# swami1995/diff-qp-mpc

Hardware: AMD Instinct MI355X
Metric: QPs/sec (fwd+bwd), batch=4096 n=3 m=3 T=5 (higher is better)
Workload: dtype f64; 1 GPU; random dense QP family R (SURVEY 8d), configs[0] shape at the BASELINE metric batch: B=4096/GPU nz=30 nineq=30 neq=15; global_batch=4096, n_state=3, n_ctrl=3, T=5, parallelism=batch-shard x1, termination=batch (the reference's batch-coupled rule, parity-safe)

## Files before the change

diff-qp-mpc_amd/_lib.py:

```python
import ctypes
import os
import re

import torch

from . import _build


class dqp_dims(ctypes.Structure):
    _fields_ = [("nbatch", ctypes.c_int32), ("nz", ctypes.c_int32), ("nineq", ctypes.c_int32),
                ("neq", ctypes.c_int32),
                ("stride_Q", ctypes.c_int64), ("stride_p", ctypes.c_int64),
                ("stride_G", ctypes.c_int64), ("stride_h", ctypes.c_int64),
                ("stride_A", ctypes.c_int64), ("stride_b", ctypes.c_int64)]


class dqp_opts(ctypes.Structure):
    _fields_ = [("eps", ctypes.c_double), ("stall_tol", ctypes.c_double),
                ("max_iter", ctypes.c_int32),
                ("not_improved_lim", ctypes.c_int32), ("flags", ctypes.c_uint32),
                ("reserved", ctypes.c_int32),
                ("dyn_id", ctypes.c_int32), ("dyn_T", ctypes.c_int32), ("dyn_dt", ctypes.c_double),
                ("dyn_x0", ctypes.c_void_p)]


DQP_OK = 0
DQP_FLAG_DENSE_BACKWARD = 1
DQP_FLAG_GENERIC_ONLY = 2
DQP_FLAG_NO_NULLSPACE = 4
DQP_FLAG_RIC_GLOBAL_WS = 64
DQP_FLAG_BACKWARD_CTX = 8
DQP_FLAG_BATCH_TERMINATION = 16
DQP_FLAG_HISTORY_ONLY = 32
DQP_FLAG_STRICT_GET_STEP = 128
DQP_FLAG_STAGEWISE = 256
DQP_STATUS_Q_NOT_PD = 1
DQP_STATUS_A_RANK_DEF = 2
DQP_MAX_DIM = 64
DQP_MAX_DIM_LARGE = 512
SHARED_GRAD_KC = 64


class dqp_al_mpc_dims(ctypes.Structure):
    _fields_ = [("nbatch", ctypes.c_int32), ("n_state", ctypes.c_int32), ("n_ctrl", ctypes.c_int32),
                ("T", ctypes.c_int32)]


class dqp_al_bounds(ctypes.Structure):
    _fields_ = [("lower", ctypes.c_void_p), ("upper", ctypes.c_void_p), ("stride_b", ctypes.c_int64),
                ("stride_t", ctypes.c_int64)]


class dqp_al_dims(ctypes.Structure):
    _fields_ = [("nbatch", ctypes.c_int32), ("nz", ctypes.c_int32), ("ncon", ctypes.c_int32),
                ("reserved", ctypes.c_int32)]


class dqp_mpc_dims(ctypes.Structure):
    _fields_ = [("nbatch", ctypes.c_int32), ("n_state", ctypes.c_int32), ("n_ctrl", ctypes.c_int32),
                ("T", ctypes.c_int32), ("has_bounds", ctypes.c_int32), ("dyn_id", ctypes.c_int32),
                ("n_state_host", ctypes.c_int32)]


class dqp_deq_dims(ctypes.Structure):
    _fields_ = [("nrows", ctypes.c_int32), ("hdim", ctypes.c_int32)]


class dqp_trace_record(ctypes.Structure):
# ... 139 lines not shown
```

diff-qp-mpc_amd/csrc/dqp_common.h:

```cpp
#ifndef DQP_COMMON_H_
#define DQP_COMMON_H_
#include <hip/hip_runtime.h>
#include <stdint.h>

#include "../../include/dqp.h"
#include "dqp_trace.h"

namespace dqp {

constexpr int WAVE = 64;

struct KParams {
    const double *Q, *p, *G, *h, *A, *b;
    long long sQ, sp, sG, sh, sA, sb;
    double *zhat, *lam, *nu, *slack, *best_resid;
    const double *zin, *lamin, *nuin, *slackin, *gin;
    double *dQ, *dp, *dG, *dh, *dA, *db;
    int32_t *info;
    double *workspace;
    unsigned long long *stamps;
    int B, N, M, E;
    int ldz, ldm, lde, ldt;
    double eps, stallTol;
    int maxIter, notImprovedLim;
    unsigned flags;
    double *hist;
    const int32_t *cap;
    int histIters;
    int dynId, dynT, dynN, dynM;
    double dynDt;
    const double *dynX0;
    const double *mC, *mc, *mF, *mf, *mx0, *mul, *muu;
    double *mdC, *mdc, *mdF, *mdf, *mdx0;
    int mn, mm, mT;
    double *snap;
    const double *histIn;
    const double *extRy;
    int itBegin, itEnd;
};

__host__ __device__ inline long long mpc_bound_stride_b(const KParams &P) { return P.sG; }
__host__ __device__ inline long long mpc_bound_stride_t(const KParams &P) { return P.sh; }
inline bool mpc_bounds_strided(const KParams &P) { return P.sG != 0 || P.sh != 0; }
inline void mpc_set_bounds(KParams &P, const dqp_al_bounds *b)
{
    P.mul = b->lower; P.muu = b->upper; P.sG = b->stride_b; P.sh = b->stride_t;
}

constexpr int TERM_HDR = 8;

constexpr int TERM_MAXIT = 64;
constexpr int TERM_ACC_BYTES = 3 * 8 + TERM_HDR * 4;

__device__ __forceinline__ void hist_put(const KParams &P, long long qp, int it, double resid, double mu)
{
    double2 *h = reinterpret_cast<double2 *>(P.hist) + (long long)it * P.B + qp;
    *h = make_double2(resid, mu);
}
__device__ __forceinline__ void hist_fill(const KParams &P, long long qp, int iters)
{
    const double nan = __builtin_nan("");
    for (int it = iters; it < P.histIters; ++it)
        reinterpret_cast<double2 *>(P.hist)[(long long)it * P.B + qp] = make_double2(nan, nan);
}
__device__ __forceinline__ void term_zero_acc(const KParams &P)
{
    if (P.hist && blockIdx.x == 0) {
        unsigned *a = reinterpret_cast<unsigned *>(P.hist + (long long)P.B * P.histIters * 2);
        for (int i = threadIdx.x; i < TERM_ACC_BYTES / 4; i += blockDim.x) a[i] = 0u;
    }
}

__device__ __forceinline__ int rule_stop(unsigned long long ai, unsigned long long anb, unsigned long long ana, int maxIter,
                                         int notImprovedLim)
{
    int nNot = 0;
    for (int it = 0; it < maxIter; ++it) {
        if (it == 0 || ((ai >> it) & 1ull)) nNot = 0;
        else nNot += 1;
        if (nNot == notImprovedLim || !((anb >> it) & 1ull) || !((ana >> it) & 1ull)) return it + 1;
    }
    return maxIter;
}

__device__ __forceinline__ unsigned long long term_uniform(unsigned long long v)
{
    const unsigned lo = __builtin_amdgcn_readfirstlane((unsigned)v), hi = __builtin_amdgcn_readfirstlane((unsigned)(v >> 32));
    return ((unsigned long long)hi << 32) | lo;
}

template <bool SCALAR = false> __device__ __forceinline__ int term_cap(const KParams &P)
{
    const unsigned long long *m =
        reinterpret_cast<const unsigned long long *>(reinterpret_cast<const char *>(P.cap) - (TERM_ACC_BYTES - TERM_HDR * 4));
    const int c = P.cap[0];
    unsigned long long ai = m[0], anb = m[1], ana = m[2];
    if (SCALAR) {
        ai = term_uniform(ai); anb = term_uniform(anb); ana = term_uniform(ana);
        asm volatile("" : "+s"(ai), "+s"(anb), "+s"(ana));
    } else {
        asm volatile("" : "+v"(ai), "+v"(anb), "+v"(ana));
    }
    if (c > 0) return c;
    const int istar = rule_stop(ai, anb, ana, P.maxIter, P.notImprovedLim);
    if (blockIdx.x == 0 && threadIdx.x == 0) const_cast<int32_t *>(P.cap)[0] = istar;
    return istar;
}

__device__ __forceinline__ int term_best(const KParams &P, long long qp) { return P.cap[TERM_HDR + qp]; }
__device__ __forceinline__ bool term_flagged(const KParams &P, long long qp, int cap) { return term_best(P, qp) >= cap; }

size_t term_bytes(int B, int maxIter, int snapDim);
int term_decide(const KParams &P, void *term, void *stream);
int term_local_masks(const KParams &P, void *term, unsigned long long *masks, void *stream);
int term_decide_global(const KParams &P, void *term, const unsigned long long *masks, void *stream);
void term_bind_pass1(KParams &P, void *term, int snapDim);
void term_bind_pass2(KParams &P, void *term);


#ifdef DQP_STAMPS
extern unsigned long long *g_debug_stamps;
#endif
int r16_forward(const KParams &P, void *stream);
int r16_backward(const KParams &P, void *stream);
int r16n_forward(const KParams &P, void *stream);
long long r16n_workspace_doubles(int N, int M, int E);
int r16n_snapshot_doubles(int N, int M, int E);
bool stage_supported(int n_state, int n_ctrl);
bool stage_native(int n_state, int n_ctrl);
int stage_q(int n_state, int n_ctrl);
long long stage_layout_doubles(int n_state, int n_ctrl, int T);
int stage_snapshot_doubles(int n_state, int n_ctrl, int T);
long long stage_workspace_doubles(int n_state, int n_ctrl, int T, int B, bool stepped);
int stage_forward(const KParams &P, void *stream);
int stage_forward_stepped(const KParams &P, void *stream);
int stage_backward(const KParams &P, void *stream);
int stage_finish(const KParams &P, void *stream);
enum { STAGE_FORWARD = 0, STAGE_STEPPED = 1, STAGE_BACKWARD = 2 };
struct PadRegion {
    double *C, *F, *c, *tau, *g, *dc, *f, *df, *nu, *ry, *x0, *dx0, *dC, *dF;
};
long long pad_region_doubles(int n_host, int n_ctrl, int T, int B);
PadRegion pad_region(double *base, int n_host, int n_ctrl, int T, int B);
int pad_pack(int n, int n_host, int m, int T, int B, const PadRegion &R, const double *C, const double *c, const double *F,
             const double *f, const double *x0, const double *tau, const double *nu, const double *g, const double *ry,
             void *stream);
int pad_unpack(int n, int n_host, int m, int T, int B, const PadRegion &R, double *tau, double *nu, double *dC, double *dc,
               double *dF, double *df, double *dx0, void *stream);
long long big_workspace_doubles(int N, int M, int E);
bool big_fits(int N, int M, int E);
// ... 11 lines not shown
```

diff-qp-mpc_amd/csrc/dqp_mpc_qp.hip:

```cpp
#include "dqp_common.h"
#include "dqp_al_bounds.h"
#include "dqp_dyn_models.h"

using namespace dqp;

namespace {

struct Route {
    bool stage;
    bool padded;
};

struct Io {
    const double *C, *c, *F, *f, *x0;
    const dqp_mpc_bounds *bounds;
    double *tau, *lam, *nu, *slack;
    int32_t *info;
    double *best_resid;
    void *workspace, *termination;
    bool complete() const
    {
        return C && c && F && f && x0 && bounds->lower && bounds->upper && tau && lam && nu && slack && workspace;
    }
};
// ... 68 lines not shown
int forward(const dqp_mpc_dims *md, const dqp_opts *opts, KParams &P, Route rt, bool stepped, const Io &io, void *stream)
{
    int rc;
    P.mC = io.C; P.mc = io.c; P.mF = io.F; P.mf = io.f; P.mx0 = io.x0;
    mpc_set_bounds(P, io.bounds);
    P.zhat = io.tau; P.lam = io.lam; P.nu = io.nu; P.slack = io.slack; P.info = io.info; P.best_resid = io.best_resid;
    P.workspace = (double *)io.workspace;
    const bool batch = (P.flags & DQP_FLAG_BATCH_TERMINATION) != 0;
    if (batch && (!io.termination || P.maxIter > 64)) return DQP_ERR_BAD_ARG;
    const bool first = !stepped || P.itBegin == 0, last = !stepped || P.itEnd == P.maxIter;
    PadRegion R = {};
    if (rt.padded) {
        R = pad_region(P.workspace + stage_workspace_doubles(P.mn, P.mm, P.mT, P.B, stepped), P.mn, P.mm, P.mT, P.B);
        const double *ry = P.itEnd > P.itBegin ? P.extRy : nullptr;
        rc = pad_pack(md->n_state, P.mn, P.mm, P.mT, P.B, R, first ? io.C : nullptr, first ? io.c : nullptr,
                      first ? io.F : nullptr, first ? io.f : nullptr, first ? io.x0 : nullptr, nullptr, nullptr, nullptr, ry,
                      stream);
        if (rc != DQP_OK) return rc;
        P.mC = R.C; P.mc = R.c; P.mF = R.F; P.mf = R.f; P.mx0 = R.x0; P.zhat = R.tau; P.nu = R.nu;
        P.extRy = ry ? R.ry : nullptr;
    }
    auto done = [&](int r) {
        if (r != DQP_OK || !rt.padded) return r;
        return pad_unpack(md->n_state, P.mn, P.mm, P.mT, P.B, R, io.tau, last ? io.nu : nullptr, nullptr, nullptr, nullptr,
                          nullptr, nullptr, stream);
    };
    if (batch) {
        P.eps = opts ? opts->eps : 1e-12;
        term_bind_pass1(P, io.termination, snapshot_doubles(P, rt));
    }
    rc = !rt.stage ? r16n_forward(P, stream) : stepped ? stage_forward_stepped(P, stream) : stage_forward(P, stream);
    if (rc != DQP_OK) return stepped && rc == 1 ? DQP_ERR_TOO_LARGE : rc;
    if (!batch || !last || (P.flags & DQP_FLAG_HISTORY_ONLY)) return done(DQP_OK);
    if ((rc = term_decide(P, io.termination, stream)) != DQP_OK) return rc;
    term_bind_pass2(P, io.termination);
    return done(rt.stage ? stage_finish(P, stream) : r16n_forward(P, stream));
}

}

extern "C" {

__attribute__((visibility("default"))) size_t dqp_mpc_qp_termination_bytes(const dqp_mpc_dims *md, const dqp_opts *o)
{
    KParams P = {};
    size_t lds = 0;
    Route rt;
    if (!o || !(o->flags & DQP_FLAG_BATCH_TERMINATION) || mpc_params(md, o, P, lds, rt) != DQP_OK || md->nbatch <= 0) return 0;
    return term_bytes(P.B, P.maxIter, snapshot_doubles(P, rt));
}

__attribute__((visibility("default"))) int dqp_mpc_qp_supported(const dqp_mpc_dims *md)
{
    KParams P = {};
    size_t lds = 0;
    Route rt;
    return mpc_params(md, nullptr, P, lds, rt) == DQP_OK ? 1 : 0;
}

__attribute__((visibility("default"))) size_t dqp_mpc_qp_workspace_bytes(const dqp_mpc_dims *md)
{
    KParams P = {};
    size_t lds = 0;
    Route rt;
    if (mpc_params(md, nullptr, P, lds, rt) != DQP_OK || md->nbatch <= 0) return 0;
    return workspace_doubles(P, rt, false) * sizeof(double);
}

// ... 123 lines not shown
```

diff-qp-mpc_amd/csrc/dqp_pdipm.hip:

```cpp

#include <hip/hip_runtime.h>
#include <math.h>
#include <stdint.h>

#include "dqp_common.h"
#include "dqp_al_bounds.h"
#include "dqp_dyn_models.h"

using namespace dqp;

namespace {

#define WSYNC() __syncthreads()

__device__ __forceinline__ double bcast(double v, int src)
{
    int lo = __double2loint(v), hi = __double2hiint(v);
    lo = __builtin_amdgcn_readlane(lo, src);
    hi = __builtin_amdgcn_readlane(hi, src);
    return __hiloint2double(hi, lo);
}

template <int CTRL> __device__ __forceinline__ double dppd(double v)
{
// ... 575 lines not shown
            const double dni = bcast(dnu, i), ni = bcast(nu, i);
            if (inN) o[i * N + lane] = dni * zh + ni * dx;
        }
    }
    if (lane == 0 && P.info) { P.info[2 * qp] = status; P.info[2 * qp + 1] = 0; }
}

template <typename K>
int launch(K kernel, const KParams &P, size_t lds_bytes, void *stream)
{
    if (P.B == 0) return DQP_OK;
    if (lds_bytes > 64 * 1024) {
        if (hipFuncSetAttribute(reinterpret_cast<const void *>(kernel),
                                hipFuncAttributeMaxDynamicSharedMemorySize,
                                (int)lds_bytes) != hipSuccess)
            return DQP_ERR_LAUNCH;
    }
    DQP_LAUNCH(kernel, dim3(P.B), dim3(WAVE), lds_bytes, (hipStream_t)stream, P);
    return hipGetLastError() == hipSuccess ? DQP_OK : DQP_ERR_LAUNCH;
}

}

static inline bool is_big(const KParams &P) { return P.N > DQP_MAX_DIM || P.M > DQP_MAX_DIM || P.E > DQP_MAX_DIM; }

namespace dqp {

void fill_opts(const dqp_opts *o, KParams &P)
{
    P.eps = (o ? o->eps : 1e-12) * 0.1;
    P.stallTol = o ? o->stall_tol : 1e-10;
    P.maxIter = o ? o->max_iter : 20;
    P.notImprovedLim = o ? o->not_improved_lim : 3;
    P.flags = o ? o->flags : 0u;
    P.hist = nullptr; P.cap = nullptr; P.histIters = P.maxIter;
}

int fill_params(const dqp_dims *d, const dqp_opts *o, KParams &P, size_t &lds_bytes)
{
#ifdef DQP_STAMPS
    P.stamps = dqp::g_debug_stamps;
#else
    P.stamps = nullptr;
#endif
    if (!d) return DQP_ERR_BAD_ARG;
    if (d->nbatch < 0 || d->nz <= 0 || d->nineq <= 0 || d->neq < 0) return DQP_ERR_BAD_ARG;
    if (d->nz > DQP_MAX_DIM_LARGE || d->nineq > DQP_MAX_DIM_LARGE || d->neq > DQP_MAX_DIM_LARGE) return DQP_ERR_TOO_LARGE;
    P.B = d->nbatch; P.N = d->nz; P.M = d->nineq; P.E = d->neq;
    if (is_big(P)) {
        if (!big_fits(P.N, P.M, P.E)) return DQP_ERR_TOO_LARGE;
        if (o && o->dyn_id) return DQP_ERR_BAD_ARG;
        P.sQ = d->stride_Q; P.sp = d->stride_p; P.sG = d->stride_G;
        P.sh = d->stride_h; P.sA = d->stride_A; P.sb = d->stride_b;
        fill_opts(o, P);
        lds_bytes = 0;
        return DQP_OK;
    }
    P.ldz = d->nz | 1; P.ldm = d->nineq | 1; P.lde = d->neq | 1;
    P.ldt = P.ldz > P.ldm ? P.ldz : P.ldm;
    P.sQ = d->stride_Q; P.sp = d->stride_p; P.sG = d->stride_G;
    P.sh = d->stride_h; P.sA = d->stride_A; P.sb = d->stride_b;
    fill_opts(o, P);
    P.dynId = o ? o->dyn_id : 0;
    P.dynT = 0; P.dynN = 0; P.dynM = 0; P.dynDt = 0.0; P.dynX0 = nullptr;
    if (P.dynId) {
        int32_t n = 0, m = 0;
        if (dqp_dyn_sizes(P.dynId, &n, &m) != DQP_OK) return DQP_ERR_BAD_ARG;
// ... 62 lines not shown

static int bind_forward(KParams &P, const double *Q, const double *p, const double *G, const double *h, const double *A,
                        const double *b, double *zhat, double *lam, double *nu, double *slack, int32_t *info,
                        double *best_resid, void *workspace)
{
    if (!Q || !p || !G || !h || !zhat || !lam || !slack) return DQP_ERR_BAD_ARG;
    if (P.E > 0 && (!A || !b || !nu)) return DQP_ERR_BAD_ARG;
    P.Q = Q; P.p = p; P.G = G; P.h = h; P.A = A; P.b = b;
    P.zhat = zhat; P.lam = lam; P.nu = nu; P.slack = slack;
    P.info = info; P.best_resid = best_resid;
    P.workspace = (double *)workspace;
    return DQP_OK;
}

__attribute__((visibility("default"))) int
dqp_qp_forward(const dqp_dims *dims, const dqp_opts *opts, const double *Q, const double *p,
               const double *G, const double *h, const double *A, const double *b, double *zhat,
               double *lam, double *nu, double *slack, int32_t *info, double *best_resid,
               void *workspace, void *termination, void *stream)
{
    KParams P = {};
    size_t lds = 0;
    int rc = fill_params(dims, opts, P, lds);
    if (rc != DQP_OK) return rc;
    if (P.B == 0) return DQP_OK;
    if ((rc = bind_forward(P, Q, p, G, h, A, b, zhat, lam, nu, slack, info, best_resid, workspace)) != DQP_OK) return rc;
    if (!(P.flags & DQP_FLAG_BATCH_TERMINATION)) return forward_once(P, lds, workspace, stream);
    if (!termination || P.maxIter < 1 || P.maxIter > 64) return DQP_ERR_BAD_ARG;
    P.eps = opts ? opts->eps : 1e-12;
    const bool nullspace = workspace && !(P.flags & (DQP_FLAG_GENERIC_ONLY | DQP_FLAG_NO_NULLSPACE)) && !P.dynId && !is_big(P);
    term_bind_pass1(P, termination, nullspace ? r16n_snapshot_doubles(P.N, P.M, P.E) : 0);
    if ((rc = forward_once(P, lds, workspace, stream)) != DQP_OK) return rc;
    if (P.flags & DQP_FLAG_HISTORY_ONLY) return DQP_OK;
    if ((rc = term_decide(P, termination, stream)) != DQP_OK) return rc;
    term_bind_pass2(P, termination);
    return forward_once(P, lds, workspace, stream);
}

__attribute__((visibility("default"))) int
dqp_term_local_masks(const dqp_dims *dims, const dqp_opts *opts, void *termination, uint64_t *masks, void *stream)
{
    KParams P = {};
    size_t lds = 0;
    int rc = fill_params(dims, opts, P, lds);
    if (rc != DQP_OK) return rc;
    if (!(P.flags & DQP_FLAG_BATCH_TERMINATION) || !termination || !masks || P.maxIter < 1 || P.maxIter > 64)
        return DQP_ERR_BAD_ARG;
    if (P.B == 0) return hipMemsetAsync(masks, 0, 24, (hipStream_t)stream) == hipSuccess ? DQP_OK : DQP_ERR_LAUNCH;
    P.eps = opts ? opts->eps : 1e-12;
    return term_local_masks(P, termination, (unsigned long long *)masks, stream);
}

__attribute__((visibility("default"))) int
dqp_qp_forward_finish(const dqp_dims *dims, const dqp_opts *opts, const double *Q, const double *p,
                      const double *G, const double *h, const double *A, const double *b, double *zhat,
                      double *lam, double *nu, double *slack, int32_t *info, double *best_resid,
                      void *workspace, void *termination, const uint64_t *masks, void *stream)
{
    KParams P = {};
    size_t lds = 0;
    int rc = fill_params(dims, opts, P, lds);
    if (rc != DQP_OK) return rc;
    if (P.B == 0) return DQP_OK;
    if (!(P.flags & DQP_FLAG_BATCH_TERMINATION) || !termination || !masks || P.maxIter < 1 || P.maxIter > 64)
        return DQP_ERR_BAD_ARG;
    if ((rc = bind_forward(P, Q, p, G, h, A, b, zhat, lam, nu, slack, info, best_resid, workspace)) != DQP_OK) return rc;
    P.eps = opts ? opts->eps : 1e-12;
    const bool nullspace = workspace && !(P.flags & (DQP_FLAG_GENERIC_ONLY | DQP_FLAG_NO_NULLSPACE)) && !P.dynId && !is_big(P);
// ... 55 lines not shown
```

diff-qp-mpc_amd/csrc/dqp_r16n.hip:

```cpp

#include "dqp_r16_prims.h"

namespace dqp {
namespace r16n {

using namespace dqp::r16;

#ifndef DQP_PF_REFLECT
#define DQP_PF_REFLECT DQP_LDS_PREFETCH
#endif
#ifndef DQP_PF_ROWS
#define DQP_PF_ROWS DQP_LDS_PREFETCH
#endif
#ifndef DQP_PF_HEADS
#define DQP_PF_HEADS DQP_LDS_PREFETCH
#endif

template <int N_, int M_, int E_> struct Cfg {
    static constexpr int N = N_, M = M_, E = E_, R = N_ - E_;
    static constexpr int SN = slots(N_), SM = slots(M_), SR = slots(N_ - E_);
    static constexpr int SE = E_ > 0 ? slots(E_) : 1, EC = E_ > 0 ? E_ : 1;
    static constexpr bool PARK = slots(N_) >= 3;
    static constexpr bool PF = !PARK;
    static constexpr int RING = (PF && DQP_PF_TRI) ? DQP_TRI_RING : 0;
// ... 7 lines not shown
#endif
    static constexpr bool PIN = PARK || DQP_R16N_PIN_ALL;
#ifndef DQP_R16N_SPLIT_ALL
#define DQP_R16N_SPLIT_ALL 0
#endif
    static constexpr bool SPLIT = PARK || DQP_R16N_SPLIT_ALL;
#ifndef DQP_R16N_EARLY_CTX
#define DQP_R16N_EARLY_CTX 1
#endif
    static constexpr bool EARLY = DQP_R16N_EARLY_CTX;
    static constexpr int tailsz = E_ * (N_ - E_) + E_ * (E_ - 1) / 2;
    static constexpr int oLq = 0;
    static constexpr int oTl = tri(N_);
    static constexpr int oR = oTl;
    static constexpr int shared = tailsz > tri(M_) ? tailsz : tri(M_);
    static constexpr int oCp = oTl + shared;
    static constexpr int oHp = oCp + (N_ - E_);
    static constexpr int oQv = oHp + M_;
    static constexpr int oBw = oQv + N_;
    static constexpr int oBs = oBw + (N_ - E_), oBz = oBs + M_, oBc = oBz + M_;
    static constexpr int oDummy = oBc + 2;
    static constexpr int ldsQP = oDummy + 16;
    static constexpr int ldsQPpad = (ldsQP + 1) & ~1;
#ifndef DQP_R16N_STAGED
#define DQP_R16N_STAGED 0
#endif
    static constexpr bool STAGED = DQP_R16N_STAGED && 16 * N_ <= ldsQP - oTl;
    __host__ __device__ static constexpr int toff(int k) { return k * (N_ - E_) + k * (k - 1) / 2; }
    static constexpr int wTl = 0, wLq = tailsz, wG = wLq + tri(N_), wU = wG + M_ * N_;
    static constexpr int wTau = wU + E_ * E_, wRdu = wTau + E_, wRdq = wRdu + E_;
    static constexpr int wXy = wRdq + N_, wPy = wXy + E_, wW1 = wPy + E_, wDl = wW1 + E_;
    static constexpr int wsQP = wDl + 1;
    static constexpr int snapDim = (N_ - E_) + 2 * M_ + 2;
};

#define DQP_PHASE_FENCE() asm volatile("" ::: "memory")
__device__ __forceinline__ void pin(double &x) { asm volatile("" : "+v"(x) : : "memory"); }
__device__ __forceinline__ const double *relabel(const double *p)
{
    asm volatile("" : "+v"(p));
    return p;
}

template <class C> struct State {
    double Gh[C::SM][C::N];
    double LqZ[C::SN][C::R];
    double Ah[C::SE][C::N];
    double tau[C::SE];
    double rdu1[C::SE];
    double xy[C::SE];
    double py[C::SE];
    double w1[C::SE];
    double rdq[C::SN];
    double rdiag[C::SM];
    int status;
};

template <class C>
__device__ __forceinline__ void shift_down(const double (&vn)[C::SN], double (&ve)[C::SE], int r)
{
#pragma unroll
    for (int s = 0; s < C::SE; ++s) ve[s] = 0.0;
#pragma unroll
    for (int e = 0; e < C::E; ++e) {
        const double t = BC(vn, C::R + e);
        if (r == (e & 15)) ve[e >> 4] = t;
// ... 886 lines not shown
            if (inM[s]) { P.lam[qp * M + r + 16 * s] = bz[s]; P.slack[qp * M + r + 16 * s] = bs[s]; }
        if (E > 0) {
#pragma unroll
            for (int s = 0; s < SE; ++s)
                if (r + 16 * s < E) P.nu[qp * E + r + 16 * s] = yv[s];
        }
        if (r == 0) {
            if (P.info) { P.info[2 * qp] = st.status; P.info[2 * qp + 1] = iters; }
            if (P.best_resid) P.best_resid[qp] = best;
        }
    }
}

template <class C>
__global__ __launch_bounds__(64) void forward_kernel(KParams P)
{
    constexpr int N = C::N, M = C::M, E = C::E, R = C::R;
    constexpr int SN = C::SN, SM = C::SM, SE = C::SE, SR = C::SR;
    extern __shared__ __attribute__((aligned(16))) double sm[];
    const int lane = threadIdx.x, r = lane & 15, qrow = lane >> 4;
    long long qp = (long long)blockIdx.x * 4 + qrow;
    bool live = qp < P.B;
    if (!live) qp = P.B - 1;
    int maxIter = P.maxIter;
    const bool batch = (P.flags & DQP_FLAG_BATCH_TERMINATION) != 0;
    const bool strict = (P.flags & DQP_FLAG_STRICT_GET_STEP) != 0;
    if (P.cap) {
        const int cap = term_cap<true>(P);
        maxIter = min(maxIter, cap);
        live = live && term_flagged(P, qp, cap);
        if (__builtin_amdgcn_ballot_w64(live) == 0) return;
    }
    double *lds = sm + qrow * C::ldsQPpad;
    double *dummy = lds + C::oDummy + r;

    term_zero_acc(P);
    State<C> st;
    STAMP(P, 0);
    setup<C>(P, qp, r, lds, st);
    STAMP(P, 15);

    bool inM[SM], inR[SR];
#pragma unroll
    for (int s = 0; s < SM; ++s) inM[s] = r + 16 * s < M;
#pragma unroll
    for (int s = 0; s < SR; ++s) inR[s] = r + 16 * s < R;

    double T[SM][M], rdu[SM];
    double w[SR], s_[SM], z[SM];
    double cc = 1.0, delta = 0.0;
    {
        double one[SM], hp[SM], cp[SR], g[SM], gtz[SR];
#pragma unroll
        for (int s = 0; s < SM; ++s) one[s] = inM[s] ? 1.0 : 0.0;
        vec_get<SM>(lds + C::oHp, hp, M, r);
        vec_get<SR>(lds + C::oCp, cp, R, r);
        mul_Gz<C>(st, cp, g);
#pragma unroll
        for (int s = 0; s < SM; ++s) g[s] = inM[s] ? -hp[s] - g[s] : 0.0;
        __builtin_amdgcn_sched_barrier(0);
        factor_T_rhs<C>(lds, T, st.rdiag, one, rdu, g, r);
        __builtin_amdgcn_sched_barrier(0);
        mul_GzT<C>(st, g, gtz, r);
#pragma unroll
        for (int s = 0; s < SR; ++s) w[s] = inR[s] ? -cp[s] - gtz[s] : 0.0;
        double ms = INFINITY, mz = INFINITY;
// ... 31 lines not shown
#pragma unroll
            for (int s = 0; s < SR; ++s) rw[s] = inR[s] ? w[s] + cp[s] + gz[s] : 0.0;
#pragma unroll
            for (int s = 0; s < SM; ++s) rz[s] = inM[s] ? gw[s] + s_[s] - hp[s] : 0.0;
        }
        double sz = 0.0, nz2 = 0.0;
#pragma unroll
        for (int s = 0; s < SM; ++s) { sz = fma(s_[s], z[s], sz); nz2 = fma(rz[s], rz[s], nz2); }
        double nx2 = rx_norm2_partial<C>(st, lds, rw, cc * delta, r);
        sz = row_sum(sz); nz2 = row_sum(nz2); nx2 = row_sum(nx2);
        const double mu = fabs(sz * (1.0 / M));
        const double resid = sqrt(nz2) + sqrt(nx2) + M * mu;
        if (!done) {
            iters = it + 1;
            if (!have_best || resid < best) {
                nNot = 0; have_best = true; best = resid; bestc = cc;
                vec_put<SR>(lds + C::oBw, w, R, r, dummy);
                vec_put<SM>(lds + C::oBs, s_, M, r, dummy);
                vec_put<SM>(lds + C::oBz, z, M, r, dummy);
                if (P.snap && live) {
                    double *sp = P.snap + ((long long)it * P.B + qp) * C::snapDim;
#pragma unroll
                    for (int s = 0; s < SR; ++s)
                        if (inR[s]) sp[r + 16 * s] = w[s];
#pragma unroll
                    for (int s = 0; s < SM; ++s)
                        if (inM[s]) { sp[R + r + 16 * s] = s_[s]; sp[R + M + r + 16 * s] = z[s]; }
                    if (r == 0) sp[R + 2 * M] = cc;
                }
            } else {
                nNot += 1;
            }
            if (batch) {
                if (P.hist && r == 0 && live) hist_put(P, qp, it, resid, mu);
                done = !(fabs(resid) < INFINITY);
            } else if ((nNot >= P.notImprovedLim && best < P.stallTol) || best < P.eps || mu > 1e32 ||
                       !(fabs(resid) < INFINITY))
                done = true;
        }
        if (__builtin_amdgcn_ballot_w64(!done) == 0 || it + 1 >= maxIter) break;
        if (it == 1) STAMP(P, 9);

        double dza[SM], dsa[SM];
        {
            double gu[SM];
            mul_Gz<C>(st, rw, gu);
#pragma unroll
            for (int s = 0; s < SM; ++s) dza[s] = rz[s] - s_[s] - gu[s];
        }
        __builtin_amdgcn_sched_barrier(0);
        double dinv[SM];
#pragma unroll
        for (int s = 0; s < SM; ++s) dinv[s] = inM[s] ? s_[s] * frcp(z[s]) : 0.0;
        factor_T_rhs<C>(lds, T, st.rdiag, dinv, rdu, dza, r);
        if (it == 1) STAMP(P, 10);
        if (it == 1) STAMP(P, 11);
        double rzv[SM], rsv[SM];
#pragma unroll
        for (int s = 0; s < SM; ++s) {
            rzv[s] = inM[s] ? frcp(z[s]) : 0.0;
            rsv[s] = inM[s] ? frcp(s_[s]) : 0.0;
        }
        double tm = 0.0;
#pragma unroll
        for (int s = 0; s < SM; ++s) {
            dsa[s] = (-z[s] - dza[s]) * dinv[s];
            tm = fmax(tm, fmax(-dza[s] * rzv[s], -dsa[s] * rsv[s]));
// ... 21 lines not shown
        if (it == 1) STAMP(P, 12);
        tm = 0.0;
#pragma unroll
        for (int s = 0; s < SM; ++s) {
            dz[s] = dza[s] + dzc[s];
            ds[s] = fma(-rsc[s] - dzc[s], dinv[s], dsa[s]);
            tm = fmax(tm, fmax(-dz[s] * rzv[s], -ds[s] * rsv[s]));
        }
        if (strict) {
#pragma unroll
            for (int s = 0; s < SM; ++s) zero_step |= inM[s] && (dz[s] == 0.0 || ds[s] == 0.0);
            if ((__builtin_amdgcn_ballot_w64(zero_step) >> (lane & 48)) & 0xffffull) done = true;
        }
        __builtin_amdgcn_sched_barrier(0);
        double gtd[SR];
        mul_GzT<C>(st, dz, gtd, r);
        alpha = frcp(fmax(row_max(tm) * (1.0 / 0.999), 1.0));
        if (!done) {
#pragma unroll
            for (int s = 0; s < SR; ++s) {
                w[s] = fma(alpha, -rw[s] - gtd[s], w[s]);
                gz[s] = fma(alpha, gtd[s], gz[s]);
            }
#pragma unroll
            for (int s = 0; s < SM; ++s) { s_[s] = fma(alpha, ds[s], s_[s]); z[s] = fma(alpha, dz[s], z[s]); }
            cc *= (1.0 - alpha);
        }
        if (it == 1) STAMP(P, 13);
        if (it == 0) STAMP(P, 8);
    }
    STAMP(P, 7);

    if (P.hist && r == 0 && live) hist_fill(P, qp, iters);
    epilogue<C>(P, qp, r, lds, st, bestc, delta, iters, best, live, true);
    STAMP(P, 14);
}

template <class C>
__device__ __forceinline__ void load_ctx(const KParams &P, long long qp, int r, double *lds, State<C> &st)
{
    constexpr int N = C::N, M = C::M, E = C::E, R = C::R;
    constexpr int SN = C::SN, SM = C::SM, SE = C::SE;
    st.status = DQP_STATUS_OK;
    {
        const double *ws = P.workspace + qp * (long long)C::wsQP;
        CtxRegs<C::tailsz> tl;
        CtxRegs<tri(N)> lq;
        ctx_fetch<C::tailsz>(ws + C::wTl, tl, r);
        ctx_fetch<tri(N)>(ws + C::wLq, lq, r);
        ctx_stash<C::tailsz>(lds + C::oTl, tl, r);
        ctx_stash<tri(N)>(lds + C::oLq, lq, r);
#pragma unroll
        for (int s = 0; s < SM; ++s) {
            const int i = r + 16 * s, ic = i < M ? i : M - 1;
#pragma unroll
            for (int c = 0; c < N; ++c) {
                const double v = ws[C::wG + c * M + ic];
                st.Gh[s][c] = (16 * s + 15 >= M) ? mask_hi(v, i < M) : v;
            }
        }
#pragma unroll
        for (int s = 0; s < SE; ++s) {
            const int k = r + 16 * s, kc = k < E ? k : E - 1;
#pragma unroll
            for (int c = 0; c < N; ++c) st.Ah[s][c] = 0.0;
#pragma unroll
            for (int e = 0; e < E; ++e) {
                const double v = ws[C::wU + e * E + kc];
                st.Ah[s][R + e] = k < E ? v : 0.0;
            }
            const double t = ws[C::wTau + kc], u = ws[C::wRdu + kc];
            st.tau[s] = k < E ? t : 0.0;
            st.rdu1[s] = k < E ? u : 0.0;
        }
#pragma unroll
        for (int s = 0; s < SN; ++s) {
            const int i = r + 16 * s;
            const double v = ws[C::wRdq + (i < N ? i : N - 1)];
            st.rdq[s] = i < N ? v : 0.0;
        }
    }
}

template <class C>
__global__ __launch_bounds__(64) void finish_kernel(KParams P)
{
    constexpr int M = C::M, E = C::E, R = C::R;
    constexpr int SM = C::SM, SE = C::SE, SR = C::SR;
    extern __shared__ __attribute__((aligned(16))) double sm[];
    const int lane = threadIdx.x, r = lane & 15, qrow = lane >> 4;
    long long qp = (long long)blockIdx.x * 4 + qrow;
    bool live = qp < P.B;
    if (!live) qp = P.B - 1;
    const int mine = term_best(P, qp);
    const int istar = term_cap<true>(P);
    live = live && mine >= istar;
    if (__builtin_amdgcn_ballot_w64(live) == 0) return;
    const int cap = min(P.maxIter, istar);
    double *lds = sm + qrow * C::ldsQPpad;
    double *dummy = lds + C::oDummy + r;
    State<C> st;
    load_ctx<C>(P, qp, r, lds, st);
    const double *ws = P.workspace + qp * (long long)C::wsQP;
#pragma unroll
    for (int s = 0; s < SE; ++s) {
        const int k = r + 16 * s, kc = k < E ? k : (E > 0 ? E - 1 : 0);
        const double a = ws[C::wXy + kc], b = ws[C::wPy + kc], c = ws[C::wW1 + kc];
        st.xy[s] = (E > 0 && k < E) ? a : 0.0;
        st.py[s] = (E > 0 && k < E) ? b : 0.0;
        st.w1[s] = (E > 0 && k < E) ? c : 0.0;
    }
    const double delta = ws[C::wDl];
    const double2 *h = reinterpret_cast<const double2 *>(P.histIn) + qp;
    double hv[64];
#pragma unroll
    for (int it = 0; it < 64; ++it) hv[it] = h[(long long)(it < cap ? it : 0) * P.B].x;
    double best = hv[0];
    int arg = 0;
#pragma unroll
    for (int it = 1; it < 64; ++it)
        if (it < cap && hv[it] < best) { best = hv[it]; arg = it; }
    const double *sp = P.snap + ((long long)arg * P.B + qp) * C::snapDim;
    double bw[SR], bs[SM], bz[SM];
#pragma unroll
    for (int s = 0; s < SR; ++s) { const int i = r + 16 * s; const double v = sp[i < R ? i : 0]; bw[s] = i < R ? v : 0.0; }
#pragma unroll
    for (int s = 0; s < SM; ++s) {
        const int i = r + 16 * s, ic = i < M ? i : 0;
// ... 167 lines not shown
        double *o = P.dQ + qp * N * N;
#pragma unroll
        for (int i = 0; i < N; ++i) {
            const double dxi = BC(dxh, i), zi = BC(zh, i);
#pragma unroll
            for (int s = 0; s < SN; ++s)
                if (inN[s]) o[i * N + r + 16 * s] = 0.5 * (dxi * zh[s] + zi * dxh[s]);
        }
    }
    if (P.dG) {
        double *o = P.dG + qp * M * N;
#pragma unroll
        for (int i = 0; i < M; ++i) {
            const double dli = BC(dlam, i), li = BC(lam, i);
#pragma unroll
            for (int s = 0; s < SN; ++s)
                if (inN[s]) o[i * N + r + 16 * s] = dli * zh[s] + li * dxh[s];
        }
    }
    if (P.dA && E > 0) {
        double *o = P.dA + qp * E * N;
#pragma unroll
        for (int i = 0; i < E; ++i) {
            const double dni = BC(dnu, i), ni = BC(nu, i);
#pragma unroll
            for (int s = 0; s < SN; ++s)
                if (inN[s]) o[i * N + r + 16 * s] = dni * zh[s] + ni * dxh[s];
        }
    }
    if (r == 0 && P.info) { P.info[2 * qp] = st.status; P.info[2 * qp + 1] = 0; }
}

template <class C, class K>
int launch(K kernel, const KParams &P, void *stream)
{
    const size_t lds = (size_t)4 * C::ldsQPpad * sizeof(double);
    if (lds > 64 * 1024 &&
        hipFuncSetAttribute(reinterpret_cast<const void *>(kernel),
                            hipFuncAttributeMaxDynamicSharedMemorySize, (int)lds) != hipSuccess)
        return DQP_ERR_LAUNCH;
    const int blocks = (P.B + 3) / 4;
    DQP_LAUNCH(kernel, dim3(blocks), dim3(64), lds, (hipStream_t)stream, P);
    return hipGetLastError() == hipSuccess ? DQP_OK : DQP_ERR_LAUNCH;
}

}

#if !defined(DQP_R16_N) || !defined(DQP_R16_M) || !defined(DQP_R16_E)
#error "compile with -DDQP_R16_N=.. -DDQP_R16_M=.. -DDQP_R16_E=.."
#endif
#define DQP_CAT2(a, n, m, e) a##n##_##m##_##e
#define DQP_CAT(a, n, m, e) DQP_CAT2(a, n, m, e)

#ifndef DQP_R16_BWD
int DQP_CAT(r16n_forward_, DQP_R16_N, DQP_R16_M, DQP_R16_E)(const KParams &P, void *stream)
{
    using C = r16n::Cfg<DQP_R16_N, DQP_R16_M, DQP_R16_E>;
    if (P.cap && P.snap && P.histIn) return r16n::launch<C>(r16n::finish_kernel<C>, P, stream);
    return r16n::launch<C>(r16n::forward_kernel<C>, P, stream);
}
#else
int DQP_CAT(r16n_backward_, DQP_R16_N, DQP_R16_M, DQP_R16_E)(const KParams &P, void *stream)
{
    using C = r16n::Cfg<DQP_R16_N, DQP_R16_M, DQP_R16_E>;
    return r16n::launch<C>(r16n::backward_kernel<C>, P, stream);
}
#endif

}
```

diff-qp-mpc_amd/csrc/dqp_term.hip:

```cpp
#include "dqp_common.h"

namespace dqp {

namespace {

constexpr int MAXIT = TERM_MAXIT;
struct Acc {
    unsigned long long improved;
    unsigned long long notbelow;
    unsigned long long notabove;
};
static_assert(sizeof(Acc) + TERM_HDR * sizeof(int32_t) == TERM_ACC_BYTES, "layout shared with dqp_common.h");

inline size_t hist_bytes(int B, int maxIter) { return (size_t)B * maxIter * 2 * sizeof(double); }

__device__ __forceinline__ unsigned long long wave_or_u64(unsigned long long v)
{
#pragma unroll
    for (int off = 32; off > 0; off >>= 1) v |= __shfl_xor(v, off, 64);
    return v;
}

constexpr int SCAN_CHUNK = 32;
__global__ __launch_bounds__(64) void term_scan_kernel(const double2 *hist, Acc *acc, int32_t *hdr,
                                                       int B, int maxIter, double eps)
{
    const int lane = threadIdx.x;
    const long long qp = (long long)blockIdx.x * blockDim.x + lane;
    const bool live = qp < B;
    unsigned long long imp = 0ull, nb = 0ull, na = 0ull;
    if (live) {
        const double2 *h = hist + qp;
        double best = 0.0;
        int arg = 0;
        for (int it0 = 0; it0 < maxIter; it0 += SCAN_CHUNK) {
            double2 v[SCAN_CHUNK];
#pragma unroll
            for (int k = 0; k < SCAN_CHUNK; ++k) v[k] = h[(long long)min(it0 + k, maxIter - 1) * B];
#pragma unroll
            for (int k = 0; k < SCAN_CHUNK; ++k) {
                const int it = it0 + k;
                if (it < maxIter) {
                    if (it == 0) best = v[k].x;
                    else if (v[k].x < best) { best = v[k].x; arg = it; imp |= 1ull << it; }
                    if (!(best < eps)) nb |= 1ull << it;
                    if (!(v[k].y > 1e32)) na |= 1ull << it;
                }
            }
        }
        hdr[TERM_HDR + qp] = arg;
    }
    imp = wave_or_u64(imp); nb = wave_or_u64(nb); na = wave_or_u64(na);
    if (lane < 3) {
        const unsigned long long m = lane == 0 ? imp : (lane == 1 ? nb : na);
        unsigned long long *dst = lane == 0 ? &acc->improved : (lane == 1 ? &acc->notbelow : &acc->notabove);
        if (m) atomicOr(dst, m);
    }
}

__global__ __launch_bounds__(64) void term_decide_kernel(const unsigned long long *masks, int32_t *hdr, int maxIter,
                                                         int notImprovedLim)
{
    if (threadIdx.x == 0) hdr[0] = rule_stop(masks[0], masks[1], masks[2], maxIter, notImprovedLim);
}

inline Acc *acc_of(void *term, int B, int maxIter) { return (Acc *)((char *)term + hist_bytes(B, maxIter)); }
inline int32_t *hdr_of(void *term, int B, int maxIter) { return (int32_t *)((char *)acc_of(term, B, maxIter) + sizeof(Acc)); }

inline size_t snap_offset(int B, int maxIter)
{
    const size_t o = hist_bytes(B, maxIter) + sizeof(Acc) + (size_t)(TERM_HDR + B) * sizeof(int32_t);
    return (o + 15) & ~(size_t)15;
}

}

size_t term_bytes(int B, int maxIter, int snapDim)
{
    if (B <= 0 || maxIter <= 0) return 0;
    return snap_offset(B, maxIter) + (size_t)B * maxIter * (snapDim > 0 ? snapDim : 0) * sizeof(double);
}

void term_bind_pass1(KParams &P, void *term, int snapDim)
{
    P.hist = (double *)term;
    P.histIters = P.maxIter;
    P.cap = nullptr;
    P.histIn = nullptr;
    P.snap = snapDim > 0 ? (double *)((char *)term + snap_offset(P.B, P.maxIter)) : nullptr;
}

void term_bind_pass2(KParams &P, void *term)
{
    P.hist = nullptr;
    P.histIn = (const double *)term;
    P.cap = hdr_of(term, P.B, P.maxIter);
}

int term_decide(const KParams &P, void *term, void *stream)
{
    const int blocks = (P.B + 63) / 64;
    DQP_LAUNCH(term_scan_kernel, dim3(blocks), dim3(64), 0, (hipStream_t)stream,
                       (const double2 *)term, acc_of(term, P.B, P.maxIter), hdr_of(term, P.B, P.maxIter),
                       P.B, P.maxIter, P.eps);
    return hipGetLastError() == hipSuccess ? DQP_OK : DQP_ERR_LAUNCH;
}

int term_local_masks(const KParams &P, void *term, unsigned long long *masks, void *stream)
{
    const int blocks = (P.B + 63) / 64;
    DQP_LAUNCH(term_scan_kernel, dim3(blocks), dim3(64), 0, (hipStream_t)stream,
                       (const double2 *)term, acc_of(term, P.B, P.maxIter), hdr_of(term, P.B, P.maxIter),
                       P.B, P.maxIter, P.eps);
    if (hipMemcpyAsync(masks, acc_of(term, P.B, P.maxIter), 3 * sizeof(unsigned long long), hipMemcpyDeviceToDevice,
                       (hipStream_t)stream) != hipSuccess)
        return DQP_ERR_LAUNCH;
    return hipGetLastError() == hipSuccess ? DQP_OK : DQP_ERR_LAUNCH;
}

int term_decide_global(const KParams &P, void *term, const unsigned long long *masks, void *stream)
{
    DQP_LAUNCH(term_decide_kernel, dim3(1), dim3(64), 0, (hipStream_t)stream, masks,
                       hdr_of(term, P.B, P.maxIter), P.maxIter, P.notImprovedLim);
    return hipGetLastError() == hipSuccess ? DQP_OK : DQP_ERR_LAUNCH;
}

// ... 2 lines not shown
```

include/dqp.h:

```cpp
#ifndef DQP_H_
#define DQP_H_

#include <stddef.h>
#include <stdint.h>

#ifdef __cplusplus
extern "C" {
#endif

#define DQP_VERSION 303
#define DQP_MAX_DIM 64
#define DQP_MAX_DIM_LARGE 512

enum {
    DQP_OK = 0,
    DQP_ERR_BAD_ARG = -1,
    DQP_ERR_TOO_LARGE = -2,
    DQP_ERR_LAUNCH = -3,
    DQP_ERR_NO_DEVICE = -4
};

enum {
    DQP_STATUS_OK = 0,
    DQP_STATUS_Q_NOT_PD = 1,
    DQP_STATUS_A_RANK_DEF = 2
};

#define DQP_FLAG_DENSE_BACKWARD 1u

#define DQP_FLAG_GENERIC_ONLY 2u
#define DQP_FLAG_BACKWARD_CTX 8u
#define DQP_FLAG_BATCH_TERMINATION 16u
#define DQP_FLAG_HISTORY_ONLY 32u
#define DQP_FLAG_NO_NULLSPACE 4u
#define DQP_FLAG_RIC_GLOBAL_WS 64u

#define DQP_FLAG_STRICT_GET_STEP 128u

#define DQP_FLAG_STAGEWISE 256u

typedef struct dqp_dims {
    int32_t nbatch;
    int32_t nz;
    int32_t nineq;
    int32_t neq;
    int64_t stride_Q, stride_p, stride_G, stride_h, stride_A, stride_b;
} dqp_dims;

typedef struct dqp_opts {
    double eps;
    double stall_tol;
    int32_t max_iter;
    int32_t not_improved_lim;
    uint32_t flags;
    int32_t reserved;
    int32_t dyn_id;
    int32_t dyn_T;
    double dyn_dt;
    const double *dyn_x0;
} dqp_opts;

int dqp_version(void);
const char *dqp_error_string(int code);


size_t dqp_workspace_bytes(const dqp_dims *dims);

size_t dqp_termination_bytes(const dqp_dims *dims, const dqp_opts *opts);

int dqp_term_local_masks(const dqp_dims *dims, const dqp_opts *opts, void *termination, uint64_t *masks,
                         void *stream);
int dqp_qp_forward_finish(const dqp_dims *dims, const dqp_opts *opts, const double *Q, const double *p,
// ... 312 lines not shown
```

Measured before the change: 18.15 million QPs/sec.

## Fuse batch-termination scan into forward kernel tail via LDS history and per-wave slots

The forward kernel now records each problem's residual and mu history in LDS instead of global memory. At the end of the kernel it computes the per-problem termination masks and argmin, then writes wave-ORed mask slots to global memory. The finish kernel ORs those slots to decide the stopping iteration, so the separate term_scan kernel launch is skipped for small-N nullspace configs. This saves a launch and a strided history re-read, at the cost of extra LDS per block, which could reduce occupancy, and more complex sync between waves.

```diff
diff --git a/diff-qp-mpc_amd/_lib.py b/diff-qp-mpc_amd/_lib.py
--- a/diff-qp-mpc_amd/_lib.py
+++ b/diff-qp-mpc_amd/_lib.py
@@ -34,6 +34,7 @@
 DQP_FLAG_HISTORY_ONLY = 32
 DQP_FLAG_STRICT_GET_STEP = 128
 DQP_FLAG_STAGEWISE = 256
+DQP_FLAG_TERM_SCAN = 512
 DQP_STATUS_Q_NOT_PD = 1
 DQP_STATUS_A_RANK_DEF = 2
 DQP_MAX_DIM = 64
diff --git a/diff-qp-mpc_amd/csrc/dqp_common.h b/diff-qp-mpc_amd/csrc/dqp_common.h
--- a/diff-qp-mpc_amd/csrc/dqp_common.h
+++ b/diff-qp-mpc_amd/csrc/dqp_common.h
@@ -52,6 +52,67 @@
 constexpr int TERM_MAXIT = 64;
 constexpr int TERM_ACC_BYTES = 3 * 8 + TERM_HDR * 4;
 
+#ifndef DQP_TERM_SLOT_WAVES
+#define DQP_TERM_SLOT_WAVES 1024
+#endif
+constexpr unsigned TERM_FLAG_SLOTS = 1u << 31;
+constexpr bool r16n_term_lds(int N) { return (N + 15) / 16 < 3; }
+
+struct TermMasks {
+    unsigned long long improved;
+    unsigned long long notbelow;
+    unsigned long long notabove;
+    int arg;
+};
+template <int CHUNK>
+__host__ __device__ inline TermMasks term_problem_masks(const double2 *h, long long stride, int maxIter, double eps)
+{
+    TermMasks m = {0ull, 0ull, 0ull, 0};
+    double best = 0.0;
+    for (int it0 = 0; it0 < maxIter; it0 += CHUNK) {
+        double2 v[CHUNK];
+#pragma unroll
+        for (int k = 0; k < CHUNK; ++k) {
+            const int itc = it0 + k < maxIter ? it0 + k : maxIter - 1;
+            v[k] = h[(long long)itc * stride];
+        }
+#pragma unroll
+        for (int k = 0; k < CHUNK; ++k) {
+            const int it = it0 + k;
+            if (it < maxIter) {
+                if (it == 0) best = v[k].x;
+                else if (v[k].x < best) { best = v[k].x; m.arg = it; m.improved |= 1ull << it; }
+                if (!(best < eps)) m.notbelow |= 1ull << it;
+                if (!(v[k].y > 1e32)) m.notabove |= 1ull << it;
+            }
+        }
+    }
+    return m;
+}
+
+__host__ __device__ inline int term_slot_pairs(int W) { return (W + 1) >> 1; }
+__host__ __device__ inline size_t term_slot_bytes(int W) { return (size_t)3 * term_slot_pairs(W) * 16; }
+template <int ROUNDS>
+__host__ __device__ inline unsigned long long term_slot_or(const unsigned long long *slots, int W, int run, int first,
+                                                           int lane, int nlanes)
+{
+    const int np = term_slot_pairs(W);
+    const ulonglong2 *s = reinterpret_cast<const ulonglong2 *>(slots) + (long long)run * np;
+    ulonglong2 v[ROUNDS];
+    bool odd[ROUNDS];
+#pragma unroll
+    for (int k = 0; k < ROUNDS; ++k) {
+        const int j = first + lane + k * nlanes, jc = j < np ? j : np - 1;
+        v[k] = s[jc];
+        odd[k] = 2 * jc + 1 >= W;
+    }
+    unsigned long long o = 0ull;
+#pragma unroll
+    for (int k = 0; k < ROUNDS; ++k) o |= v[k].x | (odd[k] ? 0ull : v[k].y);
+    return o;
+}
+constexpr int TERM_SLOT_ROUNDS = 8;
+
 __device__ __forceinline__ void hist_put(const KParams &P, long long qp, int it, double resid, double mu)
 {
     double2 *h = reinterpret_cast<double2 *>(P.hist) + (long long)it * P.B + qp;
@@ -107,6 +168,90 @@
     return istar;
 }
 
+__device__ __forceinline__ unsigned long long term_lane(unsigned long long v, int l)
+{
+    const unsigned lo = __builtin_amdgcn_readlane((unsigned)v, l), hi = __builtin_amdgcn_readlane((unsigned)(v >> 32), l);
+    return ((unsigned long long)hi << 32) | lo;
+}
+__device__ __forceinline__ unsigned term_row_or(unsigned v)
+{
+    v |= (unsigned)__builtin_amdgcn_update_dpp((int)v, (int)v, 0x128, 0xf, 0xf, true);
+    v |= (unsigned)__builtin_amdgcn_update_dpp((int)v, (int)v, 0x124, 0xf, 0xf, true);
+    v |= (unsigned)__builtin_amdgcn_update_dpp((int)v, (int)v, 0x122, 0xf, 0xf, true);
+    v |= (unsigned)__builtin_amdgcn_update_dpp((int)v, (int)v, 0x121, 0xf, 0xf, true);
+    return v;
+}
+__device__ __forceinline__ unsigned long long term_wave_or(unsigned long long v)
+{
+    const unsigned long long w = ((unsigned long long)term_row_or((unsigned)(v >> 32)) << 32) | term_row_or((unsigned)v);
+    return term_lane(w, 0) | term_lane(w, 16) | term_lane(w, 32) | term_lane(w, 48);
+}
+
+__host__ __device__ inline size_t term_slot_offset(int B, int maxIter, int snapDim)
+{
+    return (((size_t)B * maxIter * snapDim * sizeof(double)) + 15) & ~(size_t)15;
+}
+__device__ __forceinline__ unsigned long long *term_slots(const KParams &P, int snapDim)
+{
+    return reinterpret_cast<unsigned long long *>(reinterpret_cast<char *>(P.snap) + term_slot_offset(P.B, P.maxIter, snapDim));
+}
+
+__device__ __forceinline__ void term_pass1_tail(const KParams &P, double2 *hl, int qstride, long long qp, bool live, int iters,
+                                                int snapDim)
+{
+    int lane = __builtin_amdgcn_mbcnt_hi(~0u, __builtin_amdgcn_mbcnt_lo(~0u, 0u)), maxIter = P.maxIter;
+    asm volatile("" : "+v"(lane), "+s"(maxIter));
+    const int r = lane & 15, qrow = lane >> 4;
+    double2 *mine = hl + qrow * qstride;
+    if (r == 0) {
+        const double nan = __builtin_nan("");
+        for (int it = iters; it < maxIter; ++it) mine[it] = make_double2(nan, nan);
+    }
+    {
+        const long long qp0 = (long long)blockIdx.x * 4;
+        const int q = lane & 3;
+        double2 *g = reinterpret_cast<double2 *>(P.hist) + qp0 + q;
+#pragma unroll
+        for (int k = 0; k < TERM_MAXIT / 16; ++k) {
+            const int it = (lane >> 2) + 16 * k;
+            if (it < maxIter && qp0 + q < P.B) g[(long long)it * P.B] = hl[q * qstride + it];
+        }
+    }
+    TermMasks m = {0ull, 0ull, 0ull, 0};
+    if (r == 0 && live) {
+        m = term_problem_masks<8>(mine, 1, maxIter, P.eps);
+        reinterpret_cast<int32_t *>(P.hist + (long long)P.B * P.histIters * 2)[TERM_ACC_BYTES / 4 + qp] = m.arg;
+    }
+    if (P.snap) {
+        const int W = (P.B + 3) >> 2, np = term_slot_pairs(W);
+        const unsigned long long a = term_lane(m.improved, 0) | term_lane(m.improved, 16) | term_lane(m.improved, 32) |
+                                     term_lane(m.improved, 48);
+        const unsigned long long b = term_lane(m.notbelow, 0) | term_lane(m.notbelow, 16) | term_lane(m.notbelow, 32) |
+                                     term_lane(m.notbelow, 48);
+        const unsigned long long c = term_lane(m.notabove, 0) | term_lane(m.notabove, 16) | term_lane(m.notabove, 32) |
+                                     term_lane(m.notabove, 48);
+        if (lane < 3) term_slots(P, snapDim)[(long long)lane * 2 * np + blockIdx.x] = lane == 0 ? a : (lane == 1 ? b : c);
+    }
+}
+
+__device__ __forceinline__ int term_cap_slots(const KParams &P, int snapDim)
+{
+    const int W = (P.B + 3) >> 2, np = term_slot_pairs(W), lane = threadIdx.x & 63;
+    const unsigned long long *s = term_slots(P, snapDim);
+    const int c = P.cap[0];
+    unsigned long long ai = 0ull, anb = 0ull, ana = 0ull;
+    for (int first = 0; first < np; first += 64 * TERM_SLOT_ROUNDS) {
+        ai |= term_slot_or<TERM_SLOT_ROUNDS>(s, W, 0, first, lane, 64);
+        anb |= term_slot_or<TERM_SLOT_ROUNDS>(s, W, 1, first, lane, 64);
+        ana |= term_slot_or<TERM_SLOT_ROUNDS>(s, W, 2, first, lane, 64);
+    }
+    if (c > 0) return c;
+    ai = term_wave_or(ai); anb = term_wave_or(anb); ana = term_wave_or(ana);
+    const int istar = rule_stop(ai, anb, ana, P.maxIter, P.notImprovedLim);
+    if (blockIdx.x == 0 && threadIdx.x == 0) const_cast<int32_t *>(P.cap)[0] = istar;
+    return istar;
+}
+
 __device__ __forceinline__ int term_best(const KParams &P, long long qp) { return P.cap[TERM_HDR + qp]; }
 __device__ __forceinline__ bool term_flagged(const KParams &P, long long qp, int cap) { return term_best(P, qp) >= cap; }
 
@@ -115,7 +260,8 @@
 int term_local_masks(const KParams &P, void *term, unsigned long long *masks, void *stream);
 int term_decide_global(const KParams &P, void *term, const unsigned long long *masks, void *stream);
 void term_bind_pass1(KParams &P, void *term, int snapDim);
-void term_bind_pass2(KParams &P, void *term);
+bool term_use_slots(const KParams &P);
+void term_bind_pass2(KParams &P, void *term, bool slots = false);
 
 
 #ifdef DQP_STAMPS
diff --git a/diff-qp-mpc_amd/csrc/dqp_mpc_qp.hip b/diff-qp-mpc_amd/csrc/dqp_mpc_qp.hip
--- a/diff-qp-mpc_amd/csrc/dqp_mpc_qp.hip
+++ b/diff-qp-mpc_amd/csrc/dqp_mpc_qp.hip
@@ -124,8 +124,9 @@
     rc = !rt.stage ? r16n_forward(P, stream) : stepped ? stage_forward_stepped(P, stream) : stage_forward(P, stream);
     if (rc != DQP_OK) return stepped && rc == 1 ? DQP_ERR_TOO_LARGE : rc;
     if (!batch || !last || (P.flags & DQP_FLAG_HISTORY_ONLY)) return done(DQP_OK);
-    if ((rc = term_decide(P, io.termination, stream)) != DQP_OK) return rc;
-    term_bind_pass2(P, io.termination);
+    const bool slots = !rt.stage && term_use_slots(P);
+    if (!slots && (rc = term_decide(P, io.termination, stream)) != DQP_OK) return rc;
+    term_bind_pass2(P, io.termination, slots);
     return done(rt.stage ? stage_finish(P, stream) : r16n_forward(P, stream));
 }
 
diff --git a/diff-qp-mpc_amd/csrc/dqp_pdipm.hip b/diff-qp-mpc_amd/csrc/dqp_pdipm.hip
--- a/diff-qp-mpc_amd/csrc/dqp_pdipm.hip
+++ b/diff-qp-mpc_amd/csrc/dqp_pdipm.hip
@@ -631,7 +631,7 @@
     P.stallTol = o ? o->stall_tol : 1e-10;
     P.maxIter = o ? o->max_iter : 20;
     P.notImprovedLim = o ? o->not_improved_lim : 3;
-    P.flags = o ? o->flags : 0u;
+    P.flags = (o ? o->flags : 0u) & ~TERM_FLAG_SLOTS;
     P.hist = nullptr; P.cap = nullptr; P.histIters = P.maxIter;
 }
 
@@ -760,8 +760,9 @@
     term_bind_pass1(P, termination, nullspace ? r16n_snapshot_doubles(P.N, P.M, P.E) : 0);
     if ((rc = forward_once(P, lds, workspace, stream)) != DQP_OK) return rc;
     if (P.flags & DQP_FLAG_HISTORY_ONLY) return DQP_OK;
-    if ((rc = term_decide(P, termination, stream)) != DQP_OK) return rc;
-    term_bind_pass2(P, termination);
+    const bool slots = nullspace && term_use_slots(P);
+    if (!slots && (rc = term_decide(P, termination, stream)) != DQP_OK) return rc;
+    term_bind_pass2(P, termination, slots);
     return forward_once(P, lds, workspace, stream);
 }
 
diff --git a/diff-qp-mpc_amd/csrc/dqp_r16n.hip b/diff-qp-mpc_amd/csrc/dqp_r16n.hip
--- a/diff-qp-mpc_amd/csrc/dqp_r16n.hip
+++ b/diff-qp-mpc_amd/csrc/dqp_r16n.hip
@@ -63,6 +63,11 @@
     static constexpr int wXy = wRdq + N_, wPy = wXy + E_, wW1 = wPy + E_, wDl = wW1 + E_;
     static constexpr int wsQP = wDl + 1;
     static constexpr int snapDim = (N_ - E_) + 2 * M_ + 2;
+    static constexpr bool TERM_LDS = r16n_term_lds(N_);
+    static constexpr size_t ldsWave = (size_t)4 * ldsQPpad * sizeof(double);
+    static constexpr size_t ldsHist(int maxIter) { return (size_t)4 * maxIter * sizeof(double2); }
+    static_assert(!TERM_LDS || ldsWave + ldsHist(TERM_MAXIT) <= 40 * 1024,
+                  "the history region takes a wavefront off the CU");
 };
 
 #define DQP_PHASE_FENCE() asm volatile("" ::: "memory")
@@ -1015,6 +1020,7 @@
         if (__builtin_amdgcn_ballot_w64(live) == 0) return;
     }
     double *lds = sm + qrow * C::ldsQPpad;
+    double2 *hl = reinterpret_cast<double2 *>(sm + 4 * C::ldsQPpad);
     double *dummy = lds + C::oDummy + r;
 
     term_zero_acc(P);
@@ -1112,7 +1118,14 @@
                 nNot += 1;
             }
             if (batch) {
-                if (P.hist && r == 0 && live) hist_put(P, qp, it, resid, mu);
+                if (C::TERM_LDS) {
+                    if (P.hist && r == 0 && live) {
+                        hl[qrow * P.maxIter + it] = make_double2(resid, mu);
+                        asm volatile("" :: "v"(qp));
+                    }
+                } else if (P.hist && r == 0 && live) {
+                    hist_put(P, qp, it, resid, mu);
+                }
                 done = !(fabs(resid) < INFINITY);
             } else if ((nNot >= P.notImprovedLim && best < P.stallTol) || best < P.eps || mu > 1e32 ||
                        !(fabs(resid) < INFINITY))
@@ -1200,6 +1213,7 @@
     STAMP(P, 7);
 
     if (P.hist && r == 0 && live) hist_fill(P, qp, iters);
+    if (C::TERM_LDS) { if (P.hist) term_pass1_tail(P, hl, P.maxIter, qp, live, iters, C::snapDim); }
     epilogue<C>(P, qp, r, lds, st, bestc, delta, iters, best, live, true);
     STAMP(P, 14);
 }
@@ -1261,7 +1275,7 @@
     bool live = qp < P.B;
     if (!live) qp = P.B - 1;
     const int mine = term_best(P, qp);
-    const int istar = term_cap<true>(P);
+    const int istar = (C::TERM_LDS && (P.flags & TERM_FLAG_SLOTS)) ? term_cap_slots(P, C::snapDim) : term_cap<true>(P);
     live = live && mine >= istar;
     if (__builtin_amdgcn_ballot_w64(live) == 0) return;
     const int cap = min(P.maxIter, istar);
@@ -1495,9 +1509,9 @@
 }
 
 template <class C, class K>
-int launch(K kernel, const KParams &P, void *stream)
-{
-    const size_t lds = (size_t)4 * C::ldsQPpad * sizeof(double);
+int launch(K kernel, const KParams &P, void *stream, size_t lds_extra = 0)
+{
+    const size_t lds = C::ldsWave + lds_extra;
     if (lds > 64 * 1024 &&
         hipFuncSetAttribute(reinterpret_cast<const void *>(kernel),
                             hipFuncAttributeMaxDynamicSharedMemorySize, (int)lds) != hipSuccess)
@@ -1520,7 +1534,7 @@
 {
     using C = r16n::Cfg<DQP_R16_N, DQP_R16_M, DQP_R16_E>;
     if (P.cap && P.snap && P.histIn) return r16n::launch<C>(r16n::finish_kernel<C>, P, stream);
-    return r16n::launch<C>(r16n::forward_kernel<C>, P, stream);
+    return r16n::launch<C>(r16n::forward_kernel<C>, P, stream, C::TERM_LDS && P.hist ? C::ldsHist(P.maxIter) : 0);
 }
 #else
 int DQP_CAT(r16n_backward_, DQP_R16_N, DQP_R16_M, DQP_R16_E)(const KParams &P, void *stream)
diff --git a/diff-qp-mpc_amd/csrc/dqp_term.hip b/diff-qp-mpc_amd/csrc/dqp_term.hip
--- a/diff-qp-mpc_amd/csrc/dqp_term.hip
+++ b/diff-qp-mpc_amd/csrc/dqp_term.hip
@@ -30,25 +30,9 @@
     const bool live = qp < B;
     unsigned long long imp = 0ull, nb = 0ull, na = 0ull;
     if (live) {
-        const double2 *h = hist + qp;
-        double best = 0.0;
-        int arg = 0;
-        for (int it0 = 0; it0 < maxIter; it0 += SCAN_CHUNK) {
-            double2 v[SCAN_CHUNK];
-#pragma unroll
-            for (int k = 0; k < SCAN_CHUNK; ++k) v[k] = h[(long long)min(it0 + k, maxIter - 1) * B];
-#pragma unroll
-            for (int k = 0; k < SCAN_CHUNK; ++k) {
-                const int it = it0 + k;
-                if (it < maxIter) {
-                    if (it == 0) best = v[k].x;
-                    else if (v[k].x < best) { best = v[k].x; arg = it; imp |= 1ull << it; }
-                    if (!(best < eps)) nb |= 1ull << it;
-                    if (!(v[k].y > 1e32)) na |= 1ull << it;
-                }
-            }
-        }
-        hdr[TERM_HDR + qp] = arg;
+        const TermMasks m = term_problem_masks<SCAN_CHUNK>(hist + qp, B, maxIter, eps);
+        imp = m.improved; nb = m.notbelow; na = m.notabove;
+        hdr[TERM_HDR + qp] = m.arg;
     }
     imp = wave_or_u64(imp); nb = wave_or_u64(nb); na = wave_or_u64(na);
     if (lane < 3) {
@@ -78,7 +62,13 @@
 size_t term_bytes(int B, int maxIter, int snapDim)
 {
     if (B <= 0 || maxIter <= 0) return 0;
-    return snap_offset(B, maxIter) + (size_t)B * maxIter * (snapDim > 0 ? snapDim : 0) * sizeof(double);
+    if (snapDim <= 0) return snap_offset(B, maxIter);
+    return snap_offset(B, maxIter) + term_slot_offset(B, maxIter, snapDim) + term_slot_bytes((B + 3) / 4);
+}
+
+bool term_use_slots(const KParams &P)
+{
+    return P.snap && r16n_term_lds(P.N) && !(P.flags & DQP_FLAG_TERM_SCAN) && (P.B + 3) / 4 <= DQP_TERM_SLOT_WAVES;
 }
 
 void term_bind_pass1(KParams &P, void *term, int snapDim)
@@ -90,8 +80,9 @@
     P.snap = snapDim > 0 ? (double *)((char *)term + snap_offset(P.B, P.maxIter)) : nullptr;
 }
 
-void term_bind_pass2(KParams &P, void *term)
+void term_bind_pass2(KParams &P, void *term, bool slots)
 {
+    if (slots) P.flags |= TERM_FLAG_SLOTS;
     P.hist = nullptr;
     P.histIn = (const double *)term;
     P.cap = hdr_of(term, P.B, P.maxIter);
diff --git a/include/dqp.h b/include/dqp.h
--- a/include/dqp.h
+++ b/include/dqp.h
@@ -38,6 +38,8 @@
 #define DQP_FLAG_STRICT_GET_STEP 128u
 
 #define DQP_FLAG_STAGEWISE 256u
+
+#define DQP_FLAG_TERM_SCAN 512u
 
 typedef struct dqp_dims {
     int32_t nbatch;
```

After: 17.98 million QPs/sec. Within noise of the previous version (-0.9%).
